# huakunyang/SummerTTS

Hardware: AMD Instinct MI355X
Metric: audio samples/sec (acoustic model + vocoder, phoneme ids -> int16 PCM on host), single_speaker_fast-shaped synthetic blob (higher is better)
Workload: dtype f32 (decoder trunk convs AND the reverse flow's WaveNet convs (wn_flow.hip, one-utterance calls): fp32 operands as 2 fp16 terms = 22-23 of their 24 mantissa bits, 3 fp16 MFMA products per fp32 product, f32 accumulation -- measured error in `parity`, same tolerance as the exact-fp32 leg; batches addi

## Files before the change

### include/summertts_hip.h

```cpp
#ifndef SUMMERTTS_HIP_H_
#define SUMMERTTS_HIP_H_

#include <stdint.h>

#ifdef __cplusplus
extern "C" {
#endif

typedef struct sts_engine sts_engine;

enum {
    STS_OK = 0,
    STS_EINVAL = -1,
    STS_EMODEL = -2,
    STS_EDEVICE = -3,
    STS_ESTATE = -4
};

int sts_create(const float* blob, int64_t blob_bytes, int device, sts_engine** out);
void sts_destroy(sts_engine* e);

int sts_speaker_num(const sts_engine* e);

typedef struct sts_model_info {
// ... 1 lines not shown
    int32_t vocab, hidden, inter_channels, speaker_num, gin_channels;
    int32_t samples_per_frame;
    int32_t sample_rate;
    int64_t blob_floats_consumed;
} sts_model_info;
int sts_get_info(const sts_engine* e, sts_model_info* info);

int sts_infer_ids(sts_engine* e, const int32_t* ids, int32_t n, int32_t sid, float length_scale,
                  int16_t** pcm_out, int32_t* n_out);

typedef int (*sts_chunk_cb)(void* user, const int16_t* pcm, int32_t n_samples, int32_t sample_offset);
int sts_infer_ids_stream(sts_engine* e, const int32_t* ids, int32_t n, int32_t sid, float length_scale,
                         int32_t chunk_frames, sts_chunk_cb cb, void* user, int32_t* n_total);
int sts_stream_halo_frames(const sts_engine* e);

int sts_infer_ids_batch(sts_engine* e, int32_t B, const int32_t* const* ids, const int32_t* n,
                        const int32_t* sid, const float* length_scale, int16_t** pcm_out, int32_t* n_out);

int sts_run_batch(sts_engine* e, int32_t B, const int32_t* const* ids, const int32_t* n, const int32_t* sid,
                  const float* length_scale, int32_t* n_out, int64_t* total_out);
int sts_set_host_pcm(sts_engine* e, int enable);
int sts_copy_pcm_device(sts_engine* e, void* device_dst, int64_t capacity_samples);
int sts_copy_pcm_host(sts_engine* e, int16_t* host_dst, int64_t capacity_samples);
int sts_pcm_host_view(sts_engine* e, const int16_t** pcm, int64_t* count);

int sts_set_forced_durations(sts_engine* e, const int32_t* dur, int64_t count);
int sts_set_record_taps(sts_engine* e, int enable);
int sts_get_tap(sts_engine* e, const char* name, float** data, int32_t* channels, int64_t* length);
int sts_get_durations(sts_engine* e, int32_t* dur, int64_t capacity);
int sts_set_conv_mode(sts_engine* e, int mode);
int sts_set_conv_math(sts_engine* e, int mode);

enum { STS_DBG_ATTN_BLOCK_MIN_WGS = 1,
       STS_DBG_TAIL_FUSED = 14 ,
       STS_DBG_UPS_ROWPH = 15 ,
       STS_DBG_CHAIN_STREAMS = 13 ,
       STS_DBG_H2P = 11 ,
       STS_DBG_H2P_TILE = 12 ,
       STS_DBG_MEMO_CLEAR = 10 ,
       STS_DBG_PCM_DIRECT = 9 ,
       STS_DBG_DDS_TAIL = 8 ,
       STS_DBG_ATTN_REG = 7 ,
       STS_DBG_LAUNCH_AHEAD = 6 ,
       STS_DBG_FLOW_FUSED = 5  };
int sts_debug_set(sts_engine* e, int key, int value);

typedef struct sts_profile {
    float ms_text_encoder, ms_duration, ms_flow, ms_decoder, ms_total_device;
    float ms_decoder_mfma;
    int32_t decoder_mfma_launches;
    double flops_text_encoder, flops_duration, flops_flow, flops_decoder;
    double flops_decoder_mfma;
    double bytes_decoder_min;
    int64_t frames, samples, phonemes;
    double flops_decoder_mfma_executed;
    double bytes_text_encoder, bytes_duration, bytes_flow;
    float ms_sync_wait_host;
    double flops_decoder_bf16_issued;
    int64_t conv_math_fallbacks;
    int32_t conv_math_pinned;
    int32_t launch_ahead;
    int64_t launch_ahead_misses;
    float us_host_setup;
    float us_host_enqueue;
    float us_host_tail;
} sts_profile;
// ... 59 lines not shown
```

### summertts_amd/csrc/capi.hip

```cpp
#include <stdlib.h>
#include <string.h>

#include <new>
#include <string>

#include "engine.hpp"

using namespace sts;

struct sts_engine { Engine eng; };

static thread_local std::string g_err;
static int set_err(int code, const std::string& s) { g_err = s; return code; }

extern "C" {

const char* sts_last_error(void) { return g_err.c_str(); }
void sts_free(void* p) { free(p); }

int sts_create(const float* blob, int64_t blob_bytes, int device, sts_engine** out) {
    if (!out) return set_err(STS_EINVAL, "sts_create: null out pointer");
    *out = nullptr;
    sts_engine* e = new (std::nothrow) sts_engine();
    if (!e) return set_err(STS_EDEVICE, "out of host memory");
// ... 108 lines not shown
int sts_stream_halo_frames(const sts_engine* e) {
    if (!e) return set_err(STS_EINVAL, "null engine");
    return decoder_halo_frames(e->eng.model);
}

int sts_set_forced_durations(sts_engine* e, const int32_t* dur, int64_t count) {
    if (!e) return set_err(STS_EINVAL, "null engine");
    if (!dur || count <= 0) { e->eng.have_forced = false; return STS_OK; }
    e->eng.forced_dur.assign(dur, dur + count);
    e->eng.have_forced = true;
    return STS_OK;
}

int sts_set_record_taps(sts_engine* e, int enable) { if (!e) return set_err(STS_EINVAL, "null engine"); e->eng.record_taps = enable != 0; return STS_OK; }
int sts_set_conv_math(sts_engine* e, int mode) {
    if (!e) return set_err(STS_EINVAL, "null engine");
    if (mode < 0 || mode > 3) return set_err(STS_EINVAL, "conv math: 0 = split-bf16 (default), 1 = exact fp32, 2 = split-bf16 wherever eligible, 3 = two-term fp16");
    e->eng.conv_math = mode;
    e->eng.h2_consecutive = 0; e->eng.h2_disabled = false;
    return STS_OK;
}
int sts_set_conv_mode(sts_engine* e, int mode) { if (!e) return set_err(STS_EINVAL, "null engine"); e->eng.conv_mode = mode; return STS_OK; }
int sts_debug_set(sts_engine* e, int key, int value) {
    if (!e) return set_err(STS_EINVAL, "null engine");
    switch (key) {
        case STS_DBG_ATTN_BLOCK_MIN_WGS: if (value < 1) return set_err(STS_EINVAL, "threshold must be >= 1"); e->eng.attn_block_min_wgs = value; return STS_OK;
        case STS_DBG_FLOW_FUSED: e->eng.flow_fused = value != 0; return STS_OK;
        case STS_DBG_LAUNCH_AHEAD: if (value < 0 || value > 2) return set_err(STS_EINVAL, "launch_ahead must be 0, 1 or 2"); if ((value == 2) != (e->eng.launch_ahead == 2)) { e->eng.seen_tf_.clear(); e->eng.seen_order_.clear(); } e->eng.launch_ahead = value; return STS_OK;
        case STS_DBG_H2P: e->eng.h2p = value < 0 ? 0 : (value > 4 ? 4 : value); return STS_OK;
        case STS_DBG_H2P_TILE: e->eng.h2p_tile = value; return STS_OK;
        case STS_DBG_CHAIN_STREAMS: e->eng.chain_streams_dbg = value; return STS_OK;
        case STS_DBG_TAIL_FUSED: e->eng.tail_fused = value != 0; return STS_OK;
        case STS_DBG_UPS_ROWPH: e->eng.ups_rowph = value != 0; return STS_OK;
        case STS_DBG_MEMO_CLEAR: e->eng.seen_tf_.clear(); e->eng.seen_order_.clear(); return STS_OK;
        case STS_DBG_ATTN_REG: e->eng.attn_reg = value != 0; return STS_OK;
        case STS_DBG_DDS_TAIL: e->eng.dds_tail = value != 0; return STS_OK;
        case STS_DBG_PCM_DIRECT: e->eng.pcm_direct = value != 0; return STS_OK;
        default: return set_err(STS_EINVAL, "unknown debug key");
    }
}
int sts_set_host_pcm(sts_engine* e, int enable) { if (!e) return set_err(STS_EINVAL, "null engine"); e->eng.host_pcm = enable != 0; return STS_OK; }
int sts_set_profiling(sts_engine* e, int enable) { if (!e) return set_err(STS_EINVAL, "null engine"); e->eng.profiling = enable == 2 ? 2 : (enable != 0 ? 1 : 0); return STS_OK; }

int sts_abi_version(void) { return STS_ABI_VERSION; }
int sts_build_flags(void) {
#ifdef STS_EXPERIMENTS
    return 1;
#else
    return 0;
#endif
}
int sts_get_profile_ex(const sts_engine* e, void* p, int64_t size_bytes) {
    if (!e || !p || size_bytes <= 0) return set_err(STS_EINVAL, "null argument");
    const size_t n = (size_t)size_bytes < sizeof(sts_profile) ? (size_t)size_bytes : sizeof(sts_profile);
    memcpy(p, &e->eng.prof, n);
    return STS_OK;
}
int sts_get_profile(const sts_engine* e, sts_profile* p) { return sts_get_profile_ex(e, p, (int64_t)sizeof(sts_profile)); }

int sts_get_tap(sts_engine* e, const char* name, float** data, int32_t* channels, int64_t* length) {
    if (!e || !name || !data || !channels || !length) return set_err(STS_EINVAL, "null argument");
    auto it = e->eng.taps.find(name);
    if (it == e->eng.taps.end()) return set_err(STS_ESTATE, std::string("tap not recorded: ") + name);
    const Tap& t = it->second;
    float* p = (float*)malloc(t.data.size() * sizeof(float) + 4);
    if (!p) return set_err(STS_EDEVICE, "out of host memory");
// ... 151 lines not shown
}

int sts_debug_conv_h2p(int device, const float* x, int32_t Cin, int32_t L, const float* w, const float* bias, int32_t Cout, int32_t k, int32_t dil,
                       const float* res, float in_slope, float out_slope, int tile, int members, float* y_out, float* y16_out, float* yp_out,
                       int32_t iters, float* ms_out) {
    if (!x || !w || Cin <= 0 || Cout <= 0 || L <= 0 || k <= 0 || !(k & 1) || dil < 1 || members < 1 || members > kMaxGroup) return set_err(STS_EINVAL, "bad conv arguments");
    if (Cin % 16 || Cout % 32) return set_err(STS_EINVAL, "pre-split conv: Cin % 16 == 0 and Cout % 32 == 0");
    int count = 0;
    if (hipGetDeviceCount(&count) != hipSuccess || count <= 0) return set_err(STS_EDEVICE, "no HIP device visible (no CPU fallback)");
    if (hipSetDevice(device) != hipSuccess) return set_err(STS_EDEVICE, "hipSetDevice failed");
    const int pad = dil * (k - 1) / 2;
    std::vector<float> wp((size_t)k * Cin * Cout, 0.f);
    for (int o = 0; o < Cout; o++) for (int t = 0; t < k; t++) for (int ci = 0; ci < Cin; ci++)
        wp[((size_t)t * Cin + ci) * Cout + o] = w[((size_t)o * k + t) * Cin + ci];
    std::vector<unsigned char> wb(bf3_pack(wp.data(), 1, k, Cin, Cout, nullptr, true, 1));
    float wscale = 1.0f;
    bf3_pack(wp.data(), 1, k, Cin, Cout, wb.data(), true, 1, &wscale);
    const size_t in_b = (size_t)Cin * L * 4, out_b = (size_t)Cout * L * 4;
    float *dx = nullptr, *db = nullptr, *dres = nullptr, *dres16 = nullptr; void *dxp = nullptr, *dwb = nullptr, *dtmp = nullptr; unsigned* dovf = nullptr;
    float* dy[kMaxGroup] = {}; float* dy16[kMaxGroup] = {}; void* dyp[kMaxGroup] = {};
    bool ok = hipMalloc((void**)&dx, in_b) == hipSuccess && hipMalloc(&dxp, in_b) == hipSuccess && hipMalloc(&dwb, wb.size() + 8192) == hipSuccess &&
              hipMalloc((void**)&db, (size_t)Cout * 4) == hipSuccess && hipMalloc((void**)&dovf, 64) == hipSuccess;
    if (ok && res) ok = hipMalloc((void**)&dres, out_b) == hipSuccess && hipMalloc((void**)&dres16, out_b) == hipSuccess && hipMalloc(&dtmp, out_b) == hipSuccess;
    for (int m = 0; m < members && ok; m++)
        ok = hipMalloc((void**)&dy[m], out_b) == hipSuccess && hipMalloc((void**)&dy16[m], out_b) == hipSuccess && hipMalloc(&dyp[m], out_b) == hipSuccess;
    int rc = ok ? STS_OK : set_err(STS_EDEVICE, "hipMalloc failed");
    if (rc == STS_OK) {
        (void)hipMemcpy(dx, x, in_b, hipMemcpyHostToDevice);
        (void)hipMemset(dwb, 0, wb.size() + 8192);
        (void)hipMemcpy(dwb, wb.data(), wb.size(), hipMemcpyHostToDevice);
        (void)hipMemset(db, 0, (size_t)Cout * 4);
        if (bias) (void)hipMemcpy(db, bias, (size_t)Cout * 4, hipMemcpyHostToDevice);
        (void)hipMemset(dovf, 0, 64);
        split_planes(dx, L, Cin, L, in_slope, dxp, nullptr, L, dovf, nullptr);
        if (res) {
            (void)hipMemcpy(dres, res, out_b, hipMemcpyHostToDevice);
            split_planes(dres, L, Cout, L, 1.0f, dtmp, dres16, L, nullptr, nullptr);
        }
        H2PGroup G;
        memset(&G, 0, sizeof(G));
        G.n = members; G.seg = SegView{nullptr, nullptr, 1, 0, 0, L}; G.B = 1; G.max_n = L; G.ovf = dovf;
        for (int m = 0; m < members; m++) {
            H2PArgs& a = G.g[m];
            a.xp = dxp; a.xp_ld = L; a.wb = dwb; a.wscale = wscale; a.bias = bias ? db : nullptr; a.res16 = dres16; a.res_ld = L;
            a.y = iters < 0 ? nullptr : dy[m]; a.y_ld = L; a.y16 = dy16[m]; a.y16_ld = L; a.yp = dyp[m]; a.yp_ld = L; a.yp_slope = out_slope;
            a.Cin = Cin; a.Cout = Cout; a.ntap = k; a.tap_step = dil; a.tap_off = -pad;
        }
        if (!conv_h2p_group_eligible(G)) rc = set_err(STS_EINVAL, "shape not eligible for the pre-split kernel");
        else {
            conv_h2p_group(G, nullptr, tile);
            if (iters != 0 && ms_out) {
                if (iters < 0) iters = -iters;
                hipEvent_t e0, e1;
                (void)hipEventCreate(&e0); (void)hipEventCreate(&e1);
                (void)hipDeviceSynchronize();
                (void)hipEventRecord(e0, nullptr);
                for (int it = 0; it < iters; it++) conv_h2p_group(G, nullptr, tile);
                (void)hipEventRecord(e1, nullptr);
                (void)hipEventSynchronize(e1);
                float ms = 0.f;
                (void)hipEventElapsedTime(&ms, e0, e1);
                *ms_out = ms / (float)iters;
                (void)hipEventDestroy(e0); (void)hipEventDestroy(e1);
            }
            if (hipDeviceSynchronize() != hipSuccess || hipGetLastError() != hipSuccess) rc = set_err(STS_EDEVICE, "conv kernel failed");
        }
        if (rc == STS_OK) {
            if (y_out) (void)hipMemcpy(y_out, dy[0], out_b, hipMemcpyDeviceToHost);
            std::vector<float> t16((size_t)Cout * L);
            std::vector<uint16_t> tp((size_t)Cout * L * 2);
            (void)hipMemcpy(t16.data(), dy16[0], out_b, hipMemcpyDeviceToHost);
            (void)hipMemcpy(tp.data(), dyp[0], out_b, hipMemcpyDeviceToHost);
            const size_t ps = (size_t)Cout * L;
            for (int c = 0; c < Cout / 16; c++) for (long t = 0; t < L; t++) for (int h = 0; h < 2; h++) for (int e = 0; e < 8; e++) {
// ... 94 lines not shown
```

### summertts_amd/csrc/conv_h2p.hip

```cpp
#include "conv_bf3_dev.hpp"

namespace sts {

#ifdef STS_TILE_TRACE
int tile_trace_bind_h2p(long long* buf, unsigned capacity_records) { return tile_trace_bind(buf, capacity_records); }
#endif

#define STS_LDS_PTR(p) ((__attribute__((address_space(3))) void*)(p))

template <int MW, int NW, int WM, int WN>
__device__ __forceinline__ void conv_h2p_body(const H2PArgs& a, const SegView& seg, unsigned* const ovf, const int bx, const int by, const int b, [[maybe_unused]] const int tt_member) {
    constexpr int MT = 32 * MW * WM, NT = 32 * NW * WN, NWAVE = WM * WN;
    constexpr int WIN = NT + MAX_HALO;
    constexpr int NSLOT = WIN / 32;
    constexpr int SPW = (NSLOT + NWAVE - 1) / NWAVE;
    constexpr int PLANE = WIN * 32, BUF = 2 * PLANE;
    constexpr unsigned ABLK = 2048u;
    extern __shared__ __attribute__((aligned(16))) unsigned char smem3[];
#ifdef STS_TILE_TRACE
    long long* tt_rec = tt_open(2, tt_member);
    TT_STAMP(0);
#endif
    const int len = uni(seg_len(seg, b));
    const int n0 = bx * NT;
// ... 153 lines not shown
                    for (int e = 0; e < 8; e++) t[e] = __builtin_fmaxf(v[hh * 8 + e], v[hh * 8 + e] * yslope);
                    u32x4 ph, pl;
                    split8h(t, ph, pl, amax);
                    unsigned char* d = yp + (((size_t)(cc0 + hh) * a.yp_ld + base + pos) * 32 + half * 16);
                    *(u32x4*)d = ph;
                    *(u32x4*)(d + out_ps) = pl;
                }
            }
            if (y) {
                const int n = ncol + m4;
                const bool full = n + 3 < len, any = n < len;
#pragma unroll
                for (int g = 0; g < 4; g++) {
                    float w[4] = {v[4 * g], v[4 * g + 1], v[4 * g + 2], v[4 * g + 3]};
                    quad_transpose(w, l31);
                    if (any) {
                        float* p = y + (size_t)(mbase + i * 32 + 8 * g + 4 * half + lane4) * a.y_ld + base + n;
                        if (full) *(f32x4u*)p = f32x4u{w[0], w[1], w[2], w[3]};
                        else { for (int e = 0; e < 4; e++) if (n + e < len) p[e] = w[e]; }
                    }
                }
            }
            __builtin_amdgcn_sched_barrier(0);
        });
    });
    if (amax > kH2Limit && ovf) *ovf = 1u;
#ifdef STS_TILE_TRACE
    asm volatile("s_waitcnt vmcnt(0)" ::: "memory");
    TT_STAMP(3);
    TT_CLOSE();
#endif
}

template <int MW, int NW, int WM, int WN, int WPE>
__global__ __launch_bounds__(WM* WN * 64) __attribute__((amdgpu_waves_per_eu(WPE, WPE))) void conv_h2p_group_kernel(H2PGroup G, int mtiles, int nx) {
    const TileId t = map_tile(nx, mtiles, G.B * G.n);
    if (!t.valid) return;
    const int gi = t.bz / G.B, b = t.bz - gi * G.B;
    const H2PArgs* ga = (const H2PArgs*)__builtin_amdgcn_kernarg_segment_ptr();
    conv_h2p_body<MW, NW, WM, WN>(ga[gi], G.seg, G.ovf, t.bx, t.by, b, gi);
}

template <int MW, int NW, int WM, int WN, int WPE>
static void launch_h2p(const H2PGroup& G, hipStream_t st) {
    constexpr int MT = 32 * MW * WM, NT = 32 * NW * WN;
    const int mt = (G.g[0].Cout + MT - 1) / MT;
    const int nx = (G.max_n + NT - 1) / NT;
    constexpr size_t lds = (size_t)4 * (NT + MAX_HALO) * 32;
    hipLaunchKernelGGL((conv_h2p_group_kernel<MW, NW, WM, WN, WPE>), dim3(mapped_grid(nx, mt, G.B * G.n)), dim3(WM * WN * 64), lds, st, G, mt, nx);
}

bool conv_h2p_group_eligible(const H2PGroup& G) {
    if (G.n < 1 || G.n > kMaxGroup || G.max_n <= 0 || G.B <= 0) return false;
    for (int i = 0; i < G.n; i++) {
        const H2PArgs& a = G.g[i];
        if (!a.xp || !a.wb || (!a.y && !a.y16 && !a.yp)) return false;
        if (a.Cin % 16 != 0 || a.Cin < 32 || a.Cout % 128 != 0 || a.Cout != G.g[0].Cout || a.ntap < 1) return false;
        const int span = (a.ntap - 1) * a.tap_step;
        if (a.tap_step < 1 || span > MAX_HALO) return false;
        if ((double)a.xp_ld * 32.0 >= 2.0e9) return false;
    }
    return true;
}

#ifndef H2P_TILES
#define H2P_TILES 0x7ff
#endif
static int pick_h2p_tile(const H2PGroup& G) {
    const long n128 = (long)((G.max_n + 127) / 128) * (G.g[0].Cout / 128) * G.B * G.n;
    return n128 >= 768 ? 3 : 0;
}

void conv_h2p_group(const H2PGroup& Gin, hipStream_t st, int tile) {
    H2PGroup G = Gin;
    if (G.max_n <= 0 || G.B <= 0) return;
    for (int i = 1; i < G.n; i++)
        for (int j = i; j > 0 && (long)G.g[j].ntap * G.g[j].Cin > (long)G.g[j - 1].ntap * G.g[j - 1].Cin; j--) {
            H2PArgs t = G.g[j]; G.g[j] = G.g[j - 1]; G.g[j - 1] = t;
        }
    if (tile < 0 || tile > 10 || !((H2P_TILES >> tile) & 1)) tile = pick_h2p_tile(G);
    switch (tile) {
#if (H2P_TILES >> 1) & 1
        case 1: launch_h2p<2, 4, 2, 1, 2>(G, st); break;
#endif
#if (H2P_TILES >> 2) & 1
        case 2: launch_h2p<4, 2, 1, 2, 2>(G, st); break;
#endif
#if (H2P_TILES >> 3) & 1
        case 3: launch_h2p<2, 4, 2, 2, 2>(G, st); break;
#endif
#if (H2P_TILES >> 4) & 1
        case 4: launch_h2p<4, 2, 1, 4, 2>(G, st); break;
#endif
#if (H2P_TILES >> 5) & 1
        case 5: launch_h2p<4, 4, 1, 4, 1>(G, st); break;
#endif
#if (H2P_TILES >> 6) & 1
        case 6: launch_h2p<4, 4, 1, 2, 1>(G, st); break;
#endif
#if (H2P_TILES >> 7) & 1
        case 7: launch_h2p<4, 4, 1, 1, 1>(G, st); break;
#endif
#if (H2P_TILES >> 8) & 1
        case 8: launch_h2p<2, 4, 1, 1, 2>(G, st); break;
#endif
#if (H2P_TILES >> 9) & 1
        case 9: launch_h2p<2, 2, 1, 1, 3>(G, st); break;
#endif
#if (H2P_TILES >> 10) & 1
        case 10: launch_h2p<4, 2, 1, 1, 2>(G, st); break;
#endif
        default: launch_h2p<2, 2, 2, 2, 3>(G, st); break;
    }
}

__global__ __launch_bounds__(256) void split_planes_kernel(const float* x, long x_ld, int C, long n, float slope, unsigned char* planes, float* x16, long out_ld, unsigned* ovf) {
    const int lane = threadIdx.x & 63, wave = threadIdx.x >> 6;
    const int l31 = lane & 31, half = lane >> 5;
    const long pos = ((long)blockIdx.x * 4 + wave) * 32 + l31;
    const int c = blockIdx.y;
    if (pos >= n) return;
    const size_t ps = (size_t)C * (size_t)out_ld * 2u;
    float v[8], t[8];
#pragma unroll
    for (int e = 0; e < 8; e++) v[e] = x[(size_t)(16 * c + 8 * (e >> 2) + 4 * half + (e & 3)) * x_ld + pos];
#pragma unroll
    for (int e = 0; e < 8; e++) t[e] = __builtin_fmaxf(v[e], v[e] * slope);
    float amax = 0.f;
    u32x4 ph, pl;
    split8h(t, ph, pl, amax);
    unsigned char* d = planes + (((size_t)c * out_ld + pos) * 32 + half * 16);
    *(u32x4*)d = ph;
    *(u32x4*)(d + ps) = pl;
    if (x16) {
        float* o = x16 + (((size_t)c * out_ld + pos) * 16 + half * 8);
        *(f32x4u*)o = f32x4u{v[0], v[1], v[2], v[3]};
        *(f32x4u*)(o + 4) = f32x4u{v[4], v[5], v[6], v[7]};
    }
    if (amax > kH2Limit && ovf) *ovf = 1u;
}

void split_planes(const float* x, long x_ld, int C, long n, float slope, void* planes, float* x16, long out_ld, unsigned* ovf, hipStream_t st) {
    if (n <= 0 || C <= 0) return;
    hipLaunchKernelGGL(split_planes_kernel, dim3((unsigned)((n + 127) / 128), (unsigned)(C / 16)), dim3(256), 0, st, x, x_ld, C, n, slope, (unsigned char*)planes, x16, out_ld, ovf);
}

}
```

### summertts_amd/csrc/engine.hip

```cpp
#include "engine.hpp"
#include <time.h>
#include "knobs.hpp"
#include "../../include/tts_logger.h"

#include <algorithm>
#include <chrono>
#include <math.h>
#include <stdlib.h>
#include <string.h>
#include <thread>

namespace sts {

#define HIPCK(call)                                                                           \
    do {                                                                                      \
        hipError_t e__ = (call);                                                              \
        if (e__ != hipSuccess) return fail(STS_EDEVICE, std::string(#call) + ": " + hipGetErrorString(e__)); \
    } while (0)

Engine::~Engine() {
    if (stream) (void)hipStreamSynchronize(stream);
    free_model(model);
    if (arenaT_.base) (void)hipFree(arenaT_.base);
    if (arenaF_.base) (void)hipFree(arenaF_.base);
// ... 1023 lines not shown
                    mfma_flops_ += fl; mfma_exec_ += wino ? flw : fl; mfma_launches_ += 1;
                    continue;
                }
                if (h2p_stage) {
                    H2PGroup H1, H2;
                    memset(&H1, 0, sizeof(H1)); memset(&H2, 0, sizeof(H2));
                    H1.n = H2.n = nk; H1.seg = H2.seg = l2.seg; H1.B = H2.B = l2.nb; H1.max_n = H2.max_n = l2.max_len; H1.ovf = H2.ovf = ovf_;
                    float* const P0 = reg + (size_t)(1 + 4 * nk) * ce; float* const X0 = P0 + ce;
                    double fl = 0, f = 0;
                    for (int j = 0; j < nk; j++) {
                        const DResBlock& rb = M.rb[(size_t)i * nk + j];
                        const DConv &c1 = rb.c1[d], &c2 = rb.c2[d];
                        float *t1 = reg + (size_t)(1 + 3 * j) * ce, *pa = t1 + ce, *pb = pa + ce, *pn = reg + (size_t)(1 + 3 * nk + j) * ce;
                        float* nxt = (cur[j] == pa) ? pb : pa;
                        const bool last = d + 1 == nd0;
                        {
                            ConvOpt o1; o1.in_act = 1; o1.slope = 0.1f;
                            (void)conv_args(c1, cur[j], l2, t1, l2, o1, &f); fl += f;
                            ConvOpt o2; o2.in_act = 1; o2.slope = 0.1f; o2.res = cur[j]; o2.epi = EPI_RESADD;
                            (void)conv_args(c2, t1, l2, nxt, l2, o2, &f); fl += f;
                        }
                        H2PArgs& a1 = H1.g[j];
                        a1.xp = d == 0 ? (const void*)P0 : (const void*)pn; a1.xp_ld = l2.ld; a1.wb = c1.wh2p; a1.wscale = c1.h2_scale; a1.bias = c1.bias;
                        a1.yp = t1; a1.yp_ld = l2.ld; a1.yp_slope = 0.1f;
                        a1.Cin = c1.Cin; a1.Cout = c1.Cout; a1.ntap = c1.k; a1.tap_step = c1.dil; a1.tap_off = -c1.pad;
                        H2PArgs& a2 = H2.g[j];
                        a2.xp = t1; a2.xp_ld = l2.ld; a2.wb = c2.wh2p; a2.wscale = c2.h2_scale; a2.bias = c2.bias;
                        a2.res16 = d == 0 ? X0 : cur[j]; a2.res_ld = l2.ld;
                        if (last) { a2.y = nxt; a2.y_ld = l2.ld; }
                        else { a2.y16 = nxt; a2.y16_ld = l2.ld; a2.yp = pn; a2.yp_ld = l2.ld; a2.yp_slope = 0.1f; }
                        a2.Cin = c2.Cin; a2.Cout = c2.Cout; a2.ntap = c2.k; a2.tap_step = c2.dil; a2.tap_off = -c2.pad;
                        cur[j] = nxt;
                    }
                    if (d == 0) split_planes(bup, l2.ld, up.Cout, l2.total, 0.1f, P0, X0, l2.ld, ovf_, stream);
                    const int ht = h2p_tile < 0 ? -1 : (up.Cout == 128 ? (h2p_tile & 0xff) : ((h2p_tile >> 8) & 0xff));
                    conv_h2p_group(H1, stream, ht == 0xff ? -1 : ht);
                    conv_h2p_group(H2, stream, ht == 0xff ? -1 : ht);
                    mfma_flops_ += fl; bf16_exec_ += products() * fl; mfma_launches_ += 2;
                    continue;
                }
                ConvGroup G1, G2; G1.n = G2.n = nk;
                double fl1 = 0, fl2 = 0, f = 0;
                for (int j = 0; j < nk; j++) {
                    const DResBlock& rb = M.rb[(size_t)i * nk + j];
                    float *t1 = reg + (size_t)(1 + 3 * j) * ce, *pa = t1 + ce, *pb = pa + ce;
                    ConvOpt o1; o1.in_act = 1; o1.slope = 0.1f;
                    G1.g[j] = conv_args(rb.c1[d], cur[j], l2, t1, l2, o1, &f); fl1 += f;
                    ConvOpt o2; o2.in_act = 1; o2.slope = 0.1f; o2.res = cur[j]; o2.epi = EPI_RESADD;
                    float* nxt = (cur[j] == pa) ? pb : pa;
                    G2.g[j] = conv_args(rb.c2[d], t1, l2, nxt, l2, o2, &f); fl2 += f;
                    cur[j] = nxt;
                }
                static const char* gt = exp_env("STS_GROUP_TILE");
                const int gtile = gt && (int)strlen(gt) > i ? gt[i] - '0' : -1;
                if (per_chain) {
                    for (int j = 0; j < nk; j++) {
                        hipStream_t cs = aux_[crank[j] % kAux];
                        for (const ConvArgs* ca : {&G1.g[j], &G2.g[j]}) {
                            if (conv_math != 1 && conv_bf3_eligible(*ca)) conv_bf3(*ca, cs, -1);
                            else if (conv_mfma_eligible(*ca)) conv_mfma(*ca, cs, gtile);
                            else conv_generic(*ca, cs);
                        }
                    }
                    mfma_flops_ += fl1 + fl2; if (conv_math != 1) bf16_exec_ += products() * (fl1 + fl2); else mfma_exec_ += fl1 + fl2; mfma_launches_ += 2;
                    continue;
                }
                if ((conv_math != 1) && conv_bf3_group_eligible(G1) && conv_bf3_group_eligible(G2)) {
                    static const char* bgt = exp_env("STS_BF3_GROUP_TILE");
                    const int bt = bgt && (int)strlen(bgt) > i ? (bgt[i] >= '0' && bgt[i] <= '9' ? bgt[i] - '0' : (bgt[i] >= 'a' && bgt[i] <= 'z' ? bgt[i] - 'a' + 10 : -1)) : -1;
                    conv_bf3_group(G1, stream, bt);
// ... 285 lines not shown
```

### summertts_amd/csrc/engine.hpp

```cpp
#pragma once
#include <hip/hip_runtime.h>

#include <deque>
#include <map>
#include <unordered_map>
#include <string>
#include <vector>

#include "../../include/summertts_hip.h"
#include "kernels.hpp"
#include "model.hpp"

namespace sts {

struct Arena {
    char* base = nullptr; size_t cap = 0, used = 0; bool measuring = false;
    void* alloc(size_t bytes) {
        size_t a = (used + 255) & ~(size_t)255;
        used = a + bytes;
        if (measuring) return nullptr;
        return base + a;
    }
    template <typename T> T* get(size_t count) { return (T*)alloc(count * sizeof(T)); }
};
// ... 37 lines not shown
    float host_us_setup_ = 0, host_us_enq_ = 0;
    double host_t0_ = 0, host_t_sync_ = 0;
    bool pcm_in_host_ = false;
    const int16_t* h_pcm = nullptr;
    bool host_pcm = false;
    std::vector<int32_t> durations_h;
    std::map<std::string, Tap> taps;
    sts_profile prof{};
    std::vector<int32_t> forced_dur; bool have_forced = false;
    bool record_taps = false; int profiling = 0;
    int conv_mode = 0;
    int conv_math = 3;
    long h2_fallbacks = 0;
    int h2_consecutive = 0; bool h2_disabled = false;
    double products() const { return conv_math == 3 ? 3.0 : 6.0; }
    int pcm_direct = 1;
    int dds_tail = 1;
    int attn_reg = 1;
    int attn_block_min_wgs = 96;
    int launch_ahead = 1;
    long ahead_misses = 0;
    static constexpr size_t kMemoEntries = 1024;
    std::unordered_map<unsigned long long, long> seen_tf_; std::deque<unsigned long long> seen_order_;
    bool polite_wait = false;
    struct WaitEst { double us = 0.0; long phonemes = 0; };
    WaitEst wait_est_[2][24];
    void nap_before_wait(int which, long phonemes);
    void note_wait(int which, long phonemes, double waited_us, bool was_ready_at_wake);
    int final_sync(long phonemes);
    int ups_rowph = 1;
    int tail_fused = 1;
    int chain_streams_dbg = -1;
    int h2p = 1;
    int h2p_tile = -1;
    int flow_fused = 1;
    hipStream_t stream = nullptr;

private:
    int fail(int code, const std::string& msg) { err_ = msg; return code; }
    bool ensure(Arena& a, size_t bytes);
    bool ensure_pinned(size_t bytes);
    ConvArgs conv_args(const DConv& c, const float* x, const Lvl& lin, float* y, const Lvl& lout, const ConvOpt& o, double* flops);
    void conv(const DConv& c, const float* x, const Lvl& lin, float* y, const Lvl& lout, const ConvOpt& o);
    void ln(const DLn& l, const float* a, const float* b, const float* res, float* y, const Lvl& lv, int pre_relu, int post_gelu, int nb = 1, long b_stride = 0);
    int pick_kslices(const DConv& c, const Lvl& lout) const;
    struct SplineTail { const DConv* proj; float filter_sqrt; const float* r0; const float* r1; float* o0; float* o1; };
    float* dds(const DDds& d, float* h, float* t1, float* t2, const Lvl& lv, const DConv* pre = nullptr, const float* pre_in = nullptr,
               const float* pre_res = nullptr, const SplineTail* tail = nullptr, bool* tail_done = nullptr);
    struct RunCtx;
    int run_setup(RunCtx& c);
    int run_text_encoder(RunCtx& c);
    int run_durations(RunCtx& c);
    int run_frame_workspace(RunCtx& c);
    int run_flow(RunCtx& c);
    int run_decode(RunCtx& c, int nw, long Wtot, int maxW, int zoff0, int wlen0);
    int wait_frame_counts(RunCtx& c);
    int frame_geometry(RunCtx& c);
    int run_output(RunCtx& c);
    void tap(const char* name, const float* d, int channels, long ld, long length);
    void stage_begin(int s);
    void mark(int i);

    std::string err_;
    Arena arenaT_, arenaF_;
    char* pinned_ = nullptr; size_t pinned_cap_ = 0;
    char* pinned_pcm_ = nullptr; size_t pinned_pcm_cap_ = 0;
// ... 20 lines not shown
```

### summertts_amd/csrc/kernels.hpp

```cpp
#pragma once
#include <hip/hip_runtime.h>
#include <stdint.h>

namespace sts {

struct SegView {
    const int* off;
    const int* len;
    int scale;
    int extra;
    int ioff, ilen;
};

enum Epilogue : int {
    EPI_STORE = 0,
    EPI_RESADD = 1,
    EPI_SUB = 3,
    EPI_GATE = 4,
    EPI_RESSKIP = 5,
    EPI_TANH_PCM = 6,
};

struct ConvArgs {
    const float* x; long x_ld;
// ... 131 lines not shown
    int n, C; long ld; float slope;
    SegView seg; int B; int max_n;
    int math; unsigned* ovf;
};
bool resblock_layer_eligible(const ResLayerGroup& G);
void resblock_layer(const ResLayerGroup& G, hipStream_t st);
bool resblock_wino_eligible(const ResLayerGroup& G);
void resblock_wino(const ResLayerGroup& G, hipStream_t st);
bool conv_group_eligible(const ConvGroup& G);
bool conv_bf3_eligible(const ConvArgs& a);
bool conv_bf3_takes_sum(const ConvArgs& a);
bool conv_cout1_takes(const ConvArgs& a);
void conv_bf3(const ConvArgs& a, hipStream_t st, int tile = -1);
long conv_bf3_blocks(const ConvArgs& a);
bool conv_bf3_group_eligible(const ConvGroup& G);
void conv_bf3_group(const ConvGroup& G, hipStream_t st, int tile = -1);
size_t bf3_pack(const float* wp, int nphase, int ntap, int Cin_pad, int Cout_pad, void* dst, bool perm_k = false, int math = 0, float* wscale = nullptr);
bool resblock_bf3_eligible(const ResLayerGroup& G);
void resblock_bf3(const ResLayerGroup& G, hipStream_t st, int variant = -1);
void conv_mfma_group(const ConvGroup& G, hipStream_t st, int tile = -1);

struct H2PArgs {
    const void* xp; long xp_ld;
    const void* wb; float wscale;
    const float* bias;
    const float* res16; long res_ld;
    float* y; long y_ld;
    float* y16; long y16_ld;
    void* yp; long yp_ld; float yp_slope;
    int Cin, Cout, ntap, tap_step, tap_off;
};
struct H2PGroup { H2PArgs g[kMaxGroup]; int n; SegView seg; int B, max_n; unsigned* ovf; };
bool conv_h2p_group_eligible(const H2PGroup& G);
void conv_h2p_group(const H2PGroup& G, hipStream_t st, int tile = -1);
struct H2WArgs {
    const float* x16; long x_ld;
    const void* wu; float wscale;
    const float* bias;
    const float* res16; long res_ld;
    float* y16; long y16_ld;
    float* y; long y_ld;
    float in_slope, out_slope;
    int C, k, dil;
};
struct H2WGroup { H2WArgs g[kMaxGroup]; int n; SegView seg; int B, max_n; unsigned* ovf; };
bool conv_h2w_group_eligible(const H2WGroup& G);
void conv_h2w_group(const H2WGroup& G, hipStream_t st);
int h2w_transform_weights(const float* wp, int k, int Cin, int Cout, float* dst);
void to_x16(const float* x, long x_ld, int C, long n, float* x16, long out_ld, hipStream_t st);
void split_planes(const float* x, long x_ld, int C, long n, float slope, void* planes, float* x16, long out_ld, unsigned* ovf, hipStream_t st);
void conv_generic(const ConvArgs& a, hipStream_t st);

void embed(const int* ids, const float* emb, int vocab, int H, float scale, float* x, long ld, int total, hipStream_t st);
void layer_norm(const LnArgs& a, hipStream_t st);
void attention(const AttnArgs& a, hipStream_t st);
void add_ubias(float* y, long ld, const float* u, int C, SegView seg, int B, int max_len, hipStream_t st);
void gather_speaker(const float* emb_g, int spk_num, int gin, const int* sid, int B, float* g, hipStream_t st);
void sum_scale(float* y, const float* const* r, int count, long n, hipStream_t st);
void flip_channels(float* x, long ld, int C, long n, float* tmp, hipStream_t st);

void spline_step(const float* h, long ld, float filter_sqrt, const float* r0, const float* r1,
                 float* o0, float* o1, long n, hipStream_t st);
void durations(const float* r0, int sdp, float ea_m, float ea_logs, const float* ls, const int* forced,
               float* logw_out, int* dur, int* cum, int* frames, SegView seg, int B, hipStream_t st,
               int* host_out = nullptr, long total = 0, int seq = 0, unsigned* arrive = nullptr,
               int* len_out = nullptr, int* win_len_out = nullptr, int cap = 0);
void expand_frames(const float* m, long m_ld, const int* cum, SegView segT, SegView segF, int C,
                   float* z, long z_ld, int B, int max_frames, hipStream_t st);

void istft_spectrum(const float* sb, long ld, int rows, float* spec, long total, hipStream_t st);
void istft_ola(const float* spec, long ld, int bands, int band_rows, SegView seg_frames, float* tm, long tm_ld,
               SegView seg_tm, int B, int max_n, hipStream_t st);
void synth_fir(const float* tm, long tm_ld, SegView seg_tm, const float* fir, int ntap, int pad, float gain, float bias,
               float* wave, int16_t* pcm, SegView seg_out, int B, int max_n, hipStream_t st);
bool istft_tail_fused_ok(int bands, int ntap, int pad);
void istft_tail_fused(const float* sb, long ld, SegView seg_frames, const float* fir, int ntap, int pad, float gain, float bias, float* wave, int16_t* pcm,
                      SegView seg_out, int B, int max_n, hipStream_t st);
void quantize_pcm(const float* wave, int16_t* pcm, long n, hipStream_t st);

}
```

### summertts_amd/engine.py

```python
from __future__ import annotations

import ctypes as C
import os
import subprocess
from typing import Dict, List, Optional, Sequence

import numpy as np

_HERE = os.path.dirname(os.path.abspath(__file__))
LIB_PATH = os.environ.get("SUMMERTTS_HIP_LIB") or os.path.join(_HERE, "lib", "libsummertts_hip.so")
CSRC = os.path.join(_HERE, "csrc")


def build_library(verbose: bool = False) -> str:
    subprocess.run(["make", "-C", CSRC, "-j8"], check=True, stdout=None if verbose else subprocess.DEVNULL)
    return LIB_PATH


class ModelInfo(C.Structure):
    _fields_ = [("is_multi_speaker", C.c_int32), ("lang_type", C.c_int32), ("dur_pred_type", C.c_int32),
                ("dec_type", C.c_int32), ("vocab", C.c_int32), ("hidden", C.c_int32), ("inter_channels", C.c_int32),
                ("speaker_num", C.c_int32), ("gin_channels", C.c_int32), ("samples_per_frame", C.c_int32),
                ("sample_rate", C.c_int32), ("blob_floats_consumed", C.c_int64)]

# ... 172 lines not shown

    def profile_struct(self) -> "Profile":
        p = Profile()
        _check(self.lib, self.lib.sts_get_profile_ex(self.h, C.byref(p), C.sizeof(p)))
        return p

    def pcm_to_device_ptr(self, ptr: int, capacity: int) -> None:
        _check(self.lib, self.lib.sts_copy_pcm_device(self.h, C.c_void_p(ptr), capacity))

    def infer_batch(self, ids, sid=None, length_scale=None) -> List[np.ndarray]:
        n_out = self.run_batch(ids, sid, length_scale)
        flat = self.pcm_host()
        offs = np.concatenate([[0], np.cumsum(n_out)])
        return [flat[offs[b]:offs[b + 1]].copy() for b in range(len(n_out))]

    def set_forced_durations(self, dur: Optional[Sequence[int]]):
        if dur is None:
            _check(self.lib, self.lib.sts_set_forced_durations(self.h, None, 0))
            return
        d = np.ascontiguousarray(dur, dtype=np.int32)
        _check(self.lib, self.lib.sts_set_forced_durations(self.h, d.ctypes.data, d.size))

    def set_record_taps(self, on: bool):
        _check(self.lib, self.lib.sts_set_record_taps(self.h, 1 if on else 0))

    def set_conv_math(self, mode):
        m = {"bf16x3": 0, "f32": 1, "bf16x3_all": 2, "f16x2": 3}.get(mode, mode)
        _check(self.lib, self.lib.sts_set_conv_math(self.h, int(m)))

    def set_conv_mode(self, mode: int):
        _check(self.lib, self.lib.sts_set_conv_mode(self.h, mode))

    def debug_set(self, key: str, value: int):
        _check(self.lib, self.lib.sts_debug_set(self.h, {"attn_block_min_wgs": 1, "flow_fused": 5, "launch_ahead": 6, "attn_reg": 7, "dds_tail": 8, "pcm_direct": 9, "memo_clear": 10, "h2p": 11, "h2p_tile": 12, "chain_streams": 13, "tail_fused": 14, "ups_rowph": 15}[key], int(value)))

    def set_profiling(self, on):
        _check(self.lib, self.lib.sts_set_profiling(self.h, 2 if on == 2 else (1 if on else 0)))

    def profile(self) -> dict:
        p = Profile()
        _check(self.lib, self.lib.sts_get_profile_ex(self.h, C.byref(p), C.sizeof(p)))
        return p.as_dict()

    def tap(self, name: str) -> np.ndarray:
        ptr = C.POINTER(C.c_float)()
        ch, ln = C.c_int32(), C.c_int64()
        _check(self.lib, self.lib.sts_get_tap(self.h, name.encode(), C.byref(ptr), C.byref(ch), C.byref(ln)))
        a = np.ctypeslib.as_array(ptr, shape=(ch.value, ln.value)).copy()
        self.lib.sts_free(ptr)
        return a

    def durations(self, total_phonemes: int) -> np.ndarray:
        d = np.zeros(total_phonemes, np.int32)
        _check(self.lib, self.lib.sts_get_durations(self.h, d.ctypes.data, d.size))
        return d

    def close(self):
        if getattr(self, "h", None) is not None and self.h:
            self.lib.sts_destroy(self.h)
            self.h = None

    def __del__(self):
        try:
            self.close()
        except Exception:
            pass

# ... 224 lines not shown
```

Baseline: 67.22 million.

## Balance grouped trunk conv work by splitting the short-tap member into half-width tiles

Replaces the 2-D mapped grid of the grouped half-precision trunk conv kernel with a flat, XCD-interleaved unit grid. When the group is small relative to the CU count and the last member has fewer taps, that member runs with half-width N tiles to even out per-workgroup work. It also clamps the single-utterance length to the real segment length, both in the conv launch and in the plane-split kernel, so padding columns past the end are skipped. This adds a new template instantiation and some index arithmetic, and a mismatch between tile mapping and the actual layout would risk wrong coverage.

```diff
diff --git a/include/summertts_hip.h b/include/summertts_hip.h
--- a/include/summertts_hip.h
+++ b/include/summertts_hip.h
@@ -57,6 +57,7 @@
 int sts_set_conv_math(sts_engine* e, int mode);
 
 enum { STS_DBG_ATTN_BLOCK_MIN_WGS = 1,
+       STS_DBG_TRUNK_BALANCE = 16 ,
        STS_DBG_TAIL_FUSED = 14 ,
        STS_DBG_UPS_ROWPH = 15 ,
        STS_DBG_CHAIN_STREAMS = 13 ,
diff --git a/summertts_amd/csrc/capi.hip b/summertts_amd/csrc/capi.hip
--- a/summertts_amd/csrc/capi.hip
+++ b/summertts_amd/csrc/capi.hip
@@ -164,6 +164,7 @@
         case STS_DBG_CHAIN_STREAMS: e->eng.chain_streams_dbg = value; return STS_OK;
         case STS_DBG_TAIL_FUSED: e->eng.tail_fused = value != 0; return STS_OK;
         case STS_DBG_UPS_ROWPH: e->eng.ups_rowph = value != 0; return STS_OK;
+        case STS_DBG_TRUNK_BALANCE: e->eng.trunk_balance = value != 0; return STS_OK;
         case STS_DBG_MEMO_CLEAR: e->eng.seen_tf_.clear(); e->eng.seen_order_.clear(); return STS_OK;
         case STS_DBG_ATTN_REG: e->eng.attn_reg = value != 0; return STS_OK;
         case STS_DBG_DDS_TAIL: e->eng.dds_tail = value != 0; return STS_OK;
@@ -381,14 +382,15 @@
         (void)hipMemset(db, 0, (size_t)Cout * 4);
         if (bias) (void)hipMemcpy(db, bias, (size_t)Cout * 4, hipMemcpyHostToDevice);
         (void)hipMemset(dovf, 0, 64);
-        split_planes(dx, L, Cin, L, in_slope, dxp, nullptr, L, dovf, nullptr);
+        const SegView seg1{nullptr, nullptr, 1, 0, 0, L};
+        split_planes(dx, L, Cin, L, seg1, 1, in_slope, dxp, nullptr, L, dovf, nullptr);
         if (res) {
             (void)hipMemcpy(dres, res, out_b, hipMemcpyHostToDevice);
-            split_planes(dres, L, Cout, L, 1.0f, dtmp, dres16, L, nullptr, nullptr);
+            split_planes(dres, L, Cout, L, seg1, 1, 1.0f, dtmp, dres16, L, nullptr, nullptr);
         }
         H2PGroup G;
         memset(&G, 0, sizeof(G));
-        G.n = members; G.seg = SegView{nullptr, nullptr, 1, 0, 0, L}; G.B = 1; G.max_n = L; G.ovf = dovf;
+        G.n = members; G.seg = seg1; G.B = 1; G.max_n = L; G.ovf = dovf;
         for (int m = 0; m < members; m++) {
             H2PArgs& a = G.g[m];
             a.xp = dxp; a.xp_ld = L; a.wb = dwb; a.wscale = wscale; a.bias = bias ? db : nullptr; a.res16 = dres16; a.res_ld = L;
diff --git a/summertts_amd/csrc/conv_h2p.hip b/summertts_amd/csrc/conv_h2p.hip
--- a/summertts_amd/csrc/conv_h2p.hip
+++ b/summertts_amd/csrc/conv_h2p.hip
@@ -209,22 +209,40 @@
 #endif
 }
 
+template <int MW, int NW, int WM, int WN> constexpr bool kH2PHalf = MW == 2 && NW == 4 && WM == 2 && WN == 2;
+
 template <int MW, int NW, int WM, int WN, int WPE>
-__global__ __launch_bounds__(WM* WN * 64) __attribute__((amdgpu_waves_per_eu(WPE, WPE))) void conv_h2p_group_kernel(H2PGroup G, int mtiles, int nx) {
-    const TileId t = map_tile(nx, mtiles, G.B * G.n);
-    if (!t.valid) return;
-    const int gi = t.bz / G.B, b = t.bz - gi * G.B;
+__global__ __launch_bounds__(WM* WN * 64) __attribute__((amdgpu_waves_per_eu(WPE, WPE))) void conv_h2p_group_kernel(H2PGroup G, int mtiles, int nx, int nwide) {
+    const int id = blockIdx.x;
+    const int xcd = id & 7, slot = id >> 3;
+    const int ul = slot / mtiles;
+    const int by = slot - ul * mtiles;
+    const int unit = ul * 8 + xcd;
+    const int uw = nwide * G.B * nx;
     const H2PArgs* ga = (const H2PArgs*)__builtin_amdgcn_kernarg_segment_ptr();
-    conv_h2p_body<MW, NW, WM, WN>(ga[gi], G.seg, G.ovf, t.bx, t.by, b, gi);
+    if (unit < uw) {
+        const int bz = unit / nx, gi = bz / G.B, b = bz - gi * G.B;
+        conv_h2p_body<MW, NW, WM, WN>(ga[gi], G.seg, G.ovf, unit - bz * nx, by, b, gi);
+        return;
+    }
+    if constexpr (kH2PHalf<MW, NW, WM, WN>) {
+        const int nxn = 2 * nx, u = unit - uw;
+        const int bz = nwide * G.B + u / nxn;
+        if (bz >= G.n * G.B) return;
+        const int gi = bz / G.B, b = bz - gi * G.B;
+        conv_h2p_body<MW, NW / 2, WM, WN>(ga[gi], G.seg, G.ovf, u % nxn, by, b, gi);
+    }
 }
 
 template <int MW, int NW, int WM, int WN, int WPE>
-static void launch_h2p(const H2PGroup& G, hipStream_t st) {
+static void launch_h2p(const H2PGroup& G, hipStream_t st, int nwide) {
     constexpr int MT = 32 * MW * WM, NT = 32 * NW * WN;
+    if (!kH2PHalf<MW, NW, WM, WN>) nwide = G.n;
     const int mt = (G.g[0].Cout + MT - 1) / MT;
     const int nx = (G.max_n + NT - 1) / NT;
+    const long units = (long)G.B * (nwide * nx + (G.n - nwide) * 2 * nx);
     constexpr size_t lds = (size_t)4 * (NT + MAX_HALO) * 32;
-    hipLaunchKernelGGL((conv_h2p_group_kernel<MW, NW, WM, WN, WPE>), dim3(mapped_grid(nx, mt, G.B * G.n)), dim3(WM * WN * 64), lds, st, G, mt, nx);
+    hipLaunchKernelGGL((conv_h2p_group_kernel<MW, NW, WM, WN, WPE>), dim3((unsigned)((units + 7) / 8 * 8 * mt)), dim3(WM * WN * 64), lds, st, G, mt, nx, nwide);
 }
 
 bool conv_h2p_group_eligible(const H2PGroup& G) {
@@ -248,55 +266,69 @@
     return n128 >= 768 ? 3 : 0;
 }
 
-void conv_h2p_group(const H2PGroup& Gin, hipStream_t st, int tile) {
+static int h2p_wide_members(const H2PGroup& G, int tile, bool balance) {
+    if (!balance || tile != 3 || G.n < 2 || G.g[G.n - 1].ntap >= G.g[0].ntap) return G.n;
+    static const int ncu = [] { int d = 0, n = 0; (void)hipGetDevice(&d); return hipDeviceGetAttribute(&n, hipDeviceAttributeMultiprocessorCount, d) == hipSuccess ? n : 0; }();
+    const long wgs = (long)((G.max_n + 255) / 256) * (G.g[0].Cout / 128) * G.B * G.n;
+    return ncu > 0 && wgs <= 2L * ncu ? G.n - 1 : G.n;
+}
+
+void conv_h2p_group(const H2PGroup& Gin, hipStream_t st, int tile, bool balance) {
     H2PGroup G = Gin;
     if (G.max_n <= 0 || G.B <= 0) return;
+    if (G.B == 1 && !G.seg.off) {
+        const int len = G.seg.ilen * G.seg.scale + G.seg.extra;
+        if (len <= 0) return;
+        if (len < G.max_n) G.max_n = len;
+    }
     for (int i = 1; i < G.n; i++)
         for (int j = i; j > 0 && (long)G.g[j].ntap * G.g[j].Cin > (long)G.g[j - 1].ntap * G.g[j - 1].Cin; j--) {
             H2PArgs t = G.g[j]; G.g[j] = G.g[j - 1]; G.g[j - 1] = t;
         }
     if (tile < 0 || tile > 10 || !((H2P_TILES >> tile) & 1)) tile = pick_h2p_tile(G);
+    const int nw = h2p_wide_members(G, tile, balance);
     switch (tile) {
 #if (H2P_TILES >> 1) & 1
-        case 1: launch_h2p<2, 4, 2, 1, 2>(G, st); break;
+        case 1: launch_h2p<2, 4, 2, 1, 2>(G, st, nw); break;
 #endif
 #if (H2P_TILES >> 2) & 1
-        case 2: launch_h2p<4, 2, 1, 2, 2>(G, st); break;
+        case 2: launch_h2p<4, 2, 1, 2, 2>(G, st, nw); break;
 #endif
 #if (H2P_TILES >> 3) & 1
-        case 3: launch_h2p<2, 4, 2, 2, 2>(G, st); break;
+        case 3: launch_h2p<2, 4, 2, 2, 2>(G, st, nw); break;
 #endif
 #if (H2P_TILES >> 4) & 1
-        case 4: launch_h2p<4, 2, 1, 4, 2>(G, st); break;
+        case 4: launch_h2p<4, 2, 1, 4, 2>(G, st, nw); break;
 #endif
 #if (H2P_TILES >> 5) & 1
-        case 5: launch_h2p<4, 4, 1, 4, 1>(G, st); break;
+        case 5: launch_h2p<4, 4, 1, 4, 1>(G, st, nw); break;
 #endif
 #if (H2P_TILES >> 6) & 1
-        case 6: launch_h2p<4, 4, 1, 2, 1>(G, st); break;
+        case 6: launch_h2p<4, 4, 1, 2, 1>(G, st, nw); break;
 #endif
 #if (H2P_TILES >> 7) & 1
-        case 7: launch_h2p<4, 4, 1, 1, 1>(G, st); break;
+        case 7: launch_h2p<4, 4, 1, 1, 1>(G, st, nw); break;
 #endif
 #if (H2P_TILES >> 8) & 1
-        case 8: launch_h2p<2, 4, 1, 1, 2>(G, st); break;
+        case 8: launch_h2p<2, 4, 1, 1, 2>(G, st, nw); break;
 #endif
 #if (H2P_TILES >> 9) & 1
-        case 9: launch_h2p<2, 2, 1, 1, 3>(G, st); break;
+        case 9: launch_h2p<2, 2, 1, 1, 3>(G, st, nw); break;
 #endif
 #if (H2P_TILES >> 10) & 1
-        case 10: launch_h2p<4, 2, 1, 1, 2>(G, st); break;
-#endif
-        default: launch_h2p<2, 2, 2, 2, 3>(G, st); break;
-    }
-}
-
-__global__ __launch_bounds__(256) void split_planes_kernel(const float* x, long x_ld, int C, long n, float slope, unsigned char* planes, float* x16, long out_ld, unsigned* ovf) {
+        case 10: launch_h2p<4, 2, 1, 1, 2>(G, st, nw); break;
+#endif
+        default: launch_h2p<2, 2, 2, 2, 3>(G, st, nw); break;
+    }
+}
+
+__global__ __launch_bounds__(256) void split_planes_kernel(const float* x, long x_ld, int C, long n, SegView seg, int B, float slope, unsigned char* planes, float* x16, long out_ld, unsigned* ovf) {
     const int lane = threadIdx.x & 63, wave = threadIdx.x >> 6;
     const int l31 = lane & 31, half = lane >> 5;
     const long pos = ((long)blockIdx.x * 4 + wave) * 32 + l31;
     const int c = blockIdx.y;
-    if (pos >= n) return;
+    const long lim = B == 1 ? (long)uni(seg_start(seg, 0)) + uni(seg_len(seg, 0)) : n;
+    if (pos >= n || pos >= lim) return;
     const size_t ps = (size_t)C * (size_t)out_ld * 2u;
     float v[8], t[8];
 #pragma unroll
@@ -317,9 +349,9 @@
     if (amax > kH2Limit && ovf) *ovf = 1u;
 }
 
-void split_planes(const float* x, long x_ld, int C, long n, float slope, void* planes, float* x16, long out_ld, unsigned* ovf, hipStream_t st) {
-    if (n <= 0 || C <= 0) return;
-    hipLaunchKernelGGL(split_planes_kernel, dim3((unsigned)((n + 127) / 128), (unsigned)(C / 16)), dim3(256), 0, st, x, x_ld, C, n, slope, (unsigned char*)planes, x16, out_ld, ovf);
-}
-
-}
+void split_planes(const float* x, long x_ld, int C, long n, const SegView& seg, int B, float slope, void* planes, float* x16, long out_ld, unsigned* ovf, hipStream_t st) {
+    if (n <= 0 || C <= 0 || B <= 0) return;
+    hipLaunchKernelGGL(split_planes_kernel, dim3((unsigned)((n + 127) / 128), (unsigned)(C / 16)), dim3(256), 0, st, x, x_ld, C, n, seg, B, slope, (unsigned char*)planes, x16, out_ld, ovf);
+}
+
+}
diff --git a/summertts_amd/csrc/engine.hip b/summertts_amd/csrc/engine.hip
--- a/summertts_amd/csrc/engine.hip
+++ b/summertts_amd/csrc/engine.hip
@@ -1079,10 +1079,10 @@
                         a2.Cin = c2.Cin; a2.Cout = c2.Cout; a2.ntap = c2.k; a2.tap_step = c2.dil; a2.tap_off = -c2.pad;
                         cur[j] = nxt;
                     }
-                    if (d == 0) split_planes(bup, l2.ld, up.Cout, l2.total, 0.1f, P0, X0, l2.ld, ovf_, stream);
+                    if (d == 0) split_planes(bup, l2.ld, up.Cout, l2.total, l2.seg, l2.nb, 0.1f, P0, X0, l2.ld, ovf_, stream);
                     const int ht = h2p_tile < 0 ? -1 : (up.Cout == 128 ? (h2p_tile & 0xff) : ((h2p_tile >> 8) & 0xff));
-                    conv_h2p_group(H1, stream, ht == 0xff ? -1 : ht);
-                    conv_h2p_group(H2, stream, ht == 0xff ? -1 : ht);
+                    conv_h2p_group(H1, stream, ht == 0xff ? -1 : ht, trunk_balance != 0);
+                    conv_h2p_group(H2, stream, ht == 0xff ? -1 : ht, trunk_balance != 0);
                     mfma_flops_ += fl; bf16_exec_ += products() * fl; mfma_launches_ += 2;
                     continue;
                 }
diff --git a/summertts_amd/csrc/engine.hpp b/summertts_amd/csrc/engine.hpp
--- a/summertts_amd/csrc/engine.hpp
+++ b/summertts_amd/csrc/engine.hpp
@@ -93,6 +93,7 @@
     int tail_fused = 1;
     int chain_streams_dbg = -1;
     int h2p = 1;
+    int trunk_balance = 1;
     int h2p_tile = -1;
     int flow_fused = 1;
     hipStream_t stream = nullptr;
diff --git a/summertts_amd/csrc/kernels.hpp b/summertts_amd/csrc/kernels.hpp
--- a/summertts_amd/csrc/kernels.hpp
+++ b/summertts_amd/csrc/kernels.hpp
@@ -187,7 +187,7 @@
 };
 struct H2PGroup { H2PArgs g[kMaxGroup]; int n; SegView seg; int B, max_n; unsigned* ovf; };
 bool conv_h2p_group_eligible(const H2PGroup& G);
-void conv_h2p_group(const H2PGroup& G, hipStream_t st, int tile = -1);
+void conv_h2p_group(const H2PGroup& G, hipStream_t st, int tile = -1, bool balance = true);
 struct H2WArgs {
     const float* x16; long x_ld;
     const void* wu; float wscale;
@@ -203,7 +203,7 @@
 void conv_h2w_group(const H2WGroup& G, hipStream_t st);
 int h2w_transform_weights(const float* wp, int k, int Cin, int Cout, float* dst);
 void to_x16(const float* x, long x_ld, int C, long n, float* x16, long out_ld, hipStream_t st);
-void split_planes(const float* x, long x_ld, int C, long n, float slope, void* planes, float* x16, long out_ld, unsigned* ovf, hipStream_t st);
+void split_planes(const float* x, long x_ld, int C, long n, const SegView& seg, int B, float slope, void* planes, float* x16, long out_ld, unsigned* ovf, hipStream_t st);
 void conv_generic(const ConvArgs& a, hipStream_t st);
 
 void embed(const int* ids, const float* emb, int vocab, int H, float scale, float* x, long ld, int total, hipStream_t st);
diff --git a/summertts_amd/engine.py b/summertts_amd/engine.py
--- a/summertts_amd/engine.py
+++ b/summertts_amd/engine.py
@@ -228,7 +228,7 @@
         _check(self.lib, self.lib.sts_set_conv_mode(self.h, mode))
 
     def debug_set(self, key: str, value: int):
-        _check(self.lib, self.lib.sts_debug_set(self.h, {"attn_block_min_wgs": 1, "flow_fused": 5, "launch_ahead": 6, "attn_reg": 7, "dds_tail": 8, "pcm_direct": 9, "memo_clear": 10, "h2p": 11, "h2p_tile": 12, "chain_streams": 13, "tail_fused": 14, "ups_rowph": 15}[key], int(value)))
+        _check(self.lib, self.lib.sts_debug_set(self.h, {"attn_block_min_wgs": 1, "flow_fused": 5, "launch_ahead": 6, "attn_reg": 7, "dds_tail": 8, "pcm_direct": 9, "memo_clear": 10, "h2p": 11, "h2p_tile": 12, "chain_streams": 13, "tail_fused": 14, "ups_rowph": 15, "trunk_balance": 16}[key], int(value)))
 
     def set_profiling(self, on):
         _check(self.lib, self.lib.sts_set_profiling(self.h, 2 if on == 2 else (1 if on else 0)))
```

Result: no change. 67.47 million (median of 6 runs) (+0.4%).
